# ververica/ForSt

Measured on AMD Instinct MI355X. Metric: device-resident GiB/s checksummed (CRC32C/XXH3), 4–64 KiB blocks, 1/2/4/8 GPU, higher is better.
Workload: dtype u8; 1 GPU; C2: 1 M x 4 KiB kCRC32c compute+verify; blocks_per_gpu=1048576, blocks_total=1048576, checksum=kCRC32c, step=trailer pass (write side) + verify pass (read side), parallelism=byte-balanced block shards of one batch x1, no data-path collective

## Files before the change

forst_amd/csrc/crc32c.hip:

```cpp
#include "crc32c_tables.h"
#include "crc_lds.h"
#include "device_common.h"
#include "engine.h"
#include "stream_common.h"

namespace forst {
namespace {

constexpr uint32_t kRB = FORST_CRC_ROUND_BYTES;
constexpr uint32_t kWaves = 16;
constexpr uint32_t kThreads = kWaves * 64;
constexpr uint32_t kRep = 32;
constexpr uint32_t kOffJump = 4 * 256 * kRep;
constexpr uint32_t kOffTree = kOffJump + 1024;
constexpr uint32_t kLdsDwords = kOffTree + FORST_CRC_TREE_LEVELS * 1024;
constexpr uint32_t kSmall = 32;

static_assert(kLdsDwords * 4 <= 160 * 1024, "CRC tables must fit in LDS");

__device__ __forceinline__ uint32_t lds_at(const uint32_t* __restrict__ L,
                                           uint32_t byte_addr) {
  return L[byte_addr >> 2];
}

__device__ __forceinline__ uint32_t crc_g(const uint32_t* __restrict__ L,
                                          uint32_t lb, uint32_t v) {
  const uint32_t a0 = ((v & 0xffu) << 7) + lb;
  const uint32_t a1 = (((v >> 8) & 0xffu) << 7) + lb;
  const uint32_t a2 = (((v >> 16) & 0xffu) << 7) + lb;
  const uint32_t a3 = ((v >> 24) << 7) + lb;
  return L[(a0 >> 2)] ^ L[(a1 >> 2) + 8192] ^ L[(a2 >> 2) + 16384] ^
         L[(a3 >> 2) + 24576];
}

__device__ __forceinline__ uint32_t crc_byte(const uint32_t* __restrict__ L,
                                             uint32_t lb, uint32_t s,
                                             uint32_t byte) {
  const uint32_t a = (((s ^ byte) & 0xffu) << 7) + lb;
  return L[(a >> 2) + 24576] ^ (s >> 8);
}

__device__ __forceinline__ uint32_t crc_shift(const uint32_t* __restrict__ L,
                                              uint32_t T, uint32_t v) {
  return L[T + (v & 0xffu)] ^ L[T + 256 + ((v >> 8) & 0xffu)] ^
         L[T + 512 + ((v >> 16) & 0xffu)] ^ L[T + 768 + (v >> 24)];
}

__device__ __forceinline__ void load_seg(uint32_t (&w)[16],
                                         const uint8_t* seg) {
#pragma unroll
  for (int k = 0; k < 4; ++k) {
    const u32x4a4 v = ld16_a4(seg + 16 * k);
    w[4 * k + 0] = v.x;
    w[4 * k + 1] = v.y;
    w[4 * k + 2] = v.z;
    w[4 * k + 3] = v.w;
  }
}

__device__ __forceinline__ void load_seg_checked(uint32_t (&w)[16],
                                                 const uint8_t* seg,
                                                 uint64_t lo) {
#pragma unroll
  for (int k = 0; k < 4; ++k) {
    const uint8_t* c = seg + 16 * k;
    const uint64_t ca = reinterpret_cast<uint64_t>(c);
    if (ca >= lo) {
      const u32x4a4 v = ld16_a4(c);
      w[4 * k + 0] = v.x;
      w[4 * k + 1] = v.y;
      w[4 * k + 2] = v.z;
      w[4 * k + 3] = v.w;
    } else {
#pragma unroll
      for (int d = 0; d < 4; ++d)
        w[4 * k + d] = (ca + 4 * d >= lo) ? ld4_a4(c + 4 * d) : 0u;
    }
  }
}

__device__ __forceinline__ uint32_t wave_crc32c(const uint32_t* __restrict__ L,
                                                uint32_t lane,
                                uint32_t lb, const uint8_t* p, uint64_t len,
                                uint32_t init, uint32_t nextra, uint32_t extra,
                                uint64_t lo) {
  uint32_t s;
  if (len < kSmall) {
    s = ~init;
    for (uint32_t i = 0; i < static_cast<uint32_t>(len); ++i)
      s = crc_byte(L, lb, s, ldu8(p + i));
  } else {
    const uint64_t A = reinterpret_cast<uint64_t>(p);
    const uint64_t E = A + len;
    const uint64_t Aal = A & ~3ull;
    const uint32_t m = static_cast<uint32_t>(A & 3);
    uint64_t Wend = E & ~3ull;
    const uint64_t D = Wend - Aal;
    uint32_t R = static_cast<uint32_t>((D + kRB - 1) / kRB);
    if (R > 1 && (D % kRB) == 4) {
      Wend -= 4;
      --R;
    }
    const uint64_t Wstart = Wend - static_cast<uint64_t>(R) * kRB;
    const uint32_t hA = static_cast<uint32_t>(Aal - Wstart);
    const uint32_t LA = hA >> 6;
    const uint32_t jA = (hA >> 2) & 15u;
    const uint8_t* seg = p - static_cast<int64_t>(A - Wstart) + lane * 64;

    uint32_t w[16];
    if (Wstart >= lo)
      load_seg(w, seg);
    else
      load_seg_checked(w, seg, lo);
    s = 0;
#pragma unroll
    for (int j = 0; j < 16; ++j) {
      if (static_cast<uint32_t>(j) == jA) {
        if (m == 0) {
          const uint32_t s0 = (lane == LA) ? ~init : s;
          s = crc_g(L, lb, s0 ^ w[j]);
        } else {
          const uint32_t sn = crc_g(L, lb, s ^ w[j]);
          uint32_t sb = ~init;
          uint32_t wb = w[j] >> (8 * m);
          for (uint32_t b = m; b < 4; ++b) {
            sb = crc_byte(L, lb, sb, wb & 0xffu);
            wb >>= 8;
          }
          s = (lane == LA) ? sb : sn;
        }
      } else {
        s = crc_g(L, lb, s ^ w[j]);
      }
    }
    s = (lane < LA) ? 0u : s;

    for (uint32_t r = 1; r < R; ++r) {
      seg += kRB;
      load_seg(w, seg);
      s = crc_shift(L, kOffJump, s);
#pragma unroll
      for (int j = 0; j < 16; ++j) s = crc_g(L, lb, s ^ w[j]);
    }

#pragma unroll
    for (int k = 0; k < FORST_CRC_TREE_LEVELS; ++k) {
      const uint32_t other = __shfl_xor(s, 1 << k);
      const bool right = (lane >> k) & 1;
      const uint32_t left_v = right ? other : s;
      const uint32_t right_v = right ? s : other;
      s = crc_shift(L, kOffTree + 1024u * k, left_v) ^ right_v;
    }

    const uint8_t* t = p + (Wend - A);
    const uint32_t nt = static_cast<uint32_t>(E - Wend);
    for (uint32_t i = 0; i < nt; ++i) s = crc_byte(L, lb, s, ldu8(t + i));
  }
  if (nextra) s = crc_byte(L, lb, s, extra);
  return ~s;
}

__device__ __forceinline__ void fill_tables(uint32_t* L) {
  const uint32_t tid = threadIdx.x;
  for (uint32_t i = tid; i < 4 * 256 * kRep; i += kThreads) L[i] = kCrcG[i >> 5];
  for (uint32_t i = tid; i < 1024; i += kThreads) L[kOffJump + i] = kCrcJump[i];
  for (uint32_t i = tid; i < FORST_CRC_TREE_LEVELS * 1024; i += kThreads)
    L[kOffTree + i] = kCrcTree[i];
  __syncthreads();
}

using namespace fcrc;
constexpr uint32_t kOffA2 = 65536;
constexpr uint32_t kOffB2 = kOffA2 + 15 * 4096;
constexpr uint32_t kSeg2 = FORST_CRC2_SEG_BYTES;

__device__ __forceinline__ uint32_t unstep_m(uint32_t v, uint32_t m) {
  if (m == 0) return v;
  const uint32_t* col = kCrcUnstep + 32 * (m - 1);
  uint32_t r = 0;
  for (uint32_t i = 0; i < 32; ++i) r ^= ((v >> i) & 1u) ? col[i] : 0u;
  return r;
}

template <int MODE>
__device__ __forceinline__ bool mem_last_byte(const BlockArgs& a) {
  return MODE == kModeVerify || ((MODE == kModeCompute || MODE == kModeTrailer) && !a.last_bytes);
}

__device__ __forceinline__ uint32_t small_crc2(const uint8_t* __restrict__ Lb, const Lanes& K,
                                               const uint8_t* p, uint32_t len, uint32_t init,
                                               uint32_t nextra, uint32_t extra) {
  uint32_t s = ~init;
  const uint32_t m = static_cast<uint32_t>(reinterpret_cast<uint64_t>(p) & 3);
  uint32_t nh = (4 - m) & 3;
  nh = nh < len ? nh : len;
  uint32_t y = 0;
  for (uint32_t i = 0; i < nh; ++i) y |= ldu8(p + i) << (8 * i);
  s = step_k(Lb, K, s, y, nh);
  uint32_t i = nh;
  for (; i + 4 <= len; i += 4) s = rep_map<false>(Lb, K, s ^ ld4v(p + i));
  y = 0;
  const uint32_t nt = len - i;
  for (uint32_t j = 0; j < nt; ++j) y |= ldu8(p + i + j) << (8 * j);
  s = step_k(Lb, K, s, y, nt);
  if (nextra) s = step_k(Lb, K, s, extra & 0xffu, 1);
  return ~s;
}

constexpr uint32_t kStageW = 6144;
constexpr uint32_t kRowRound = 1024;
constexpr uint32_t kRowChain = 512;
constexpr uint32_t kLds3Bytes = kOffB2 + 4096;
constexpr uint32_t kNoBlk = 0xffffffffu;

template <uint32_t NT>
__device__ __forceinline__ void fill_tables3(uint32_t* L) {
  const uint32_t tid = threadIdx.x;
  constexpr uint32_t kN1 = (16384 + NT - 1) / NT, kN2 = (15 * 1024 + NT - 1) / NT,
                     kN3 = (1024 + NT - 1) / NT;
  uint32_t v1[kN1], v2[kN2], v3[kN3];
#pragma unroll
  for (uint32_t k = 0; k < kN1; ++k) {
    const uint32_t i = tid + k * NT;
    const uint32_t e = (i >> 6) & 255, d = i & 63, t = (d >> 3) & 3;
    v1[k] = i < 16384 ? (d < 32 ? kCrcG[t * 256 + e] : kCrcJ3[t * 256 + e]) : 0u;
  }
#pragma unroll
  for (uint32_t k = 0; k < kN2; ++k) {
    const uint32_t i = tid + k * NT;
    v2[k] = i < 15 * 1024 ? kCrcA[i] : 0u;
  }
#pragma unroll
  for (uint32_t k = 0; k < kN3; ++k) {
    const uint32_t i = tid + k * NT;
    v3[k] = i < 1024 ? kCrcB[i] : 0u;
  }
#pragma unroll
  for (uint32_t k = 0; k < kN1; ++k)
    if (tid + k * NT < 16384) L[tid + k * NT] = v1[k];
#pragma unroll
  for (uint32_t k = 0; k < kN2; ++k)
    if (tid + k * NT < 15 * 1024) L[kOffA2 / 4 + tid + k * NT] = v2[k];
#pragma unroll
  for (uint32_t k = 0; k < kN3; ++k)
    if (tid + k * NT < 1024) L[kOffB2 / 4 + tid + k * NT] = v3[k];
  __syncthreads();
}

struct CRowPos {
  uint32_t rp_lo, rp_hi;
  uint32_t tp_lo, tp_hi;
  uint32_t rel;
  uint32_t rl;
  uint32_t pk;
  __device__ __forceinline__ int64_t rp() const {
    return static_cast<int64_t>((static_cast<uint64_t>(rp_hi) << 32) | rp_lo);
  }
  __device__ __forceinline__ uint64_t tp() const {
    return (static_cast<uint64_t>(tp_hi) << 32) | tp_lo;
  }
  __device__ __forceinline__ uint32_t cA() const { return pk & 1u; }
  __device__ __forceinline__ uint32_t tA() const { return (pk >> 1) & 15u; }
  __device__ __forceinline__ uint32_t jA() const { return (pk >> 5) & 7u; }
  __device__ __forceinline__ uint32_t q() const { return (pk >> 8) & 7u; }
  __device__ __forceinline__ uint32_t nt() const { return (pk >> 11) & 3u; }
  __device__ __forceinline__ uint32_t m() const { return (pk >> 13) & 3u; }
  __device__ __forceinline__ bool valid() const { return (pk >> 15) & 1u; }
  __device__ __forceinline__ bool slow() const { return (pk >> 16) & 1u; }
  __device__ __forceinline__ bool xtra() const { return (pk >> 17) & 1u; }
  __device__ __forceinline__ uint32_t d1() const { return (pk >> 16) & 12u; }
  __device__ __forceinline__ bool r0() const { return (pk >> 20) & 1u; }
  __device__ __forceinline__ uint32_t slow_size() const { return (pk >> 24) & 15u; }
  __device__ __forceinline__ bool wait() const { return (pk >> 21) & 1u; }
  template <int MODE>
  __device__ __forceinline__ uint64_t end(bool mlb) const {
    const uint64_t t0 = tp() + 4;
    const uint64_t we = (MODE == kModeVerify || nt() > 0) ? t0 : t0 + 4;
    return we + nt() - (mlb ? 1u : 0u);
  }
};

template <int MODE>
__device__ __forceinline__ void crow_derive(const BlockArgs& a, uint64_t off, uint32_t size,
                                            CRowPos& P) {
  const bool valid = P.rel != kNoBlk && desc_in_range<MODE>(a, Desc{off, size, 0, 0});
  const uint64_t E = off + size + (mem_last_byte<MODE>(a) ? 1u : 0u);
  const uint64_t ws = off & ~3ull;
  const uint64_t we = E & ~3ull;
  const uint64_t d4 = we - ws;
  const bool xtra = MODE != kModeRaw && (d4 & (kRowRound - 1)) == 4 && d4 > kRowRound;
  uint32_t R = static_cast<uint32_t>(xtra ? d4 / kRowRound : (d4 + kRowRound - 1) / kRowRound);
  int64_t w0 = static_cast<int64_t>(we) - (xtra ? 4 : 0) - static_cast<int64_t>(R) * kRowRound;
  const uint32_t hA = static_cast<uint32_t>(static_cast<int64_t>(ws) - w0);
  const uint32_t cA = hA >> 9, tA = (hA >> 5) & 15u, jA = (hA >> 2) & 7u;
  const int64_t seg_head = static_cast<int64_t>(ws) - 4 * static_cast<int64_t>(jA);
  const uint32_t q = seg_head < 0 ? static_cast<uint32_t>(-seg_head) >> 2 : 0u;
  const uint32_t nt = static_cast<uint32_t>(E - we);
  const uint32_t m = static_cast<uint32_t>(off & 3);
  const uint64_t t0 = (nt > 0 || MODE == kModeVerify) ? we : we - 4;
  const uint32_t d1 = MODE == kModeVerify ? (nt > 0 ? 8u : 4u) : (xtra && nt > 0 ? 0u : 4u);
  const bool slow = !valid || d4 < 4 || t0 < 4;
  const uint64_t tp = slow ? off : t0 - 4;
  if (slow) {
    R = 1;
    w0 = 0;
  }
  P.rl = R;
  P.rp_lo = static_cast<uint32_t>(w0);
  P.rp_hi = static_cast<uint32_t>(static_cast<uint64_t>(w0) >> 32);
  P.tp_lo = static_cast<uint32_t>(tp);
  P.tp_hi = static_cast<uint32_t>(tp >> 32);
  P.pk = (slow ? (valid ? (size & 15u) << 24 : 0u)
               : (cA | (tA << 1) | (jA << 5) | (q << 8) | (xtra ? 1u << 17 : 0u) |
                  ((d1 >> 2) << 18))) |
         (nt << 11) | (m << 13) | (valid ? 1u << 15 : 0u) | (slow ? 1u << 16 : 0u) | (1u << 20);
}

struct CRStep {
  uint32_t w[2][8];
  uint32_t t0, t1, t2, mod, extra;
};

template <int MODE>
__device__ __forceinline__ void crow_issue(const BlockArgs& a, uint32_t lane, const CRowPos& P,
                                           uint64_t kbeg, CRStep& d) {
  const uint32_t t = lane & 15;
  int64_t s0 = P.rp() + kSeg2 * t;
  int64_t s1 = s0 + kRowChain;
  if (__ballot(s0 < 0)) {
    s0 = s0 < 0 ? 0 : s0;
    s1 = s1 < 0 ? 0 : s1;
  }
#pragma unroll
  for (uint32_t c = 0; c < 2; ++c) {
    const uint8_t* sp = a.base + (c ? s1 : s0);
#pragma unroll
    for (int q = 0; q < 2; ++q) {
      const u32x4a4 v = ld16_a4(sp + 16 * q);
      d.w[c][4 * q + 0] = v.x;
      d.w[c][4 * q + 1] = v.y;
      d.w[c][4 * q + 2] = v.z;
      d.w[c][4 * q + 3] = v.w;
    }
  }
  const bool lastr = !P.slow() && P.rl <= 1;
  const uint8_t* pb = a.base + (lastr ? P.tp() : 0);
  d.t0 = ld4_a4(pb + 4);
  d.t1 = MODE == kModeRaw ? 0u : ld4_a4(pb + P.d1());
  d.t2 = MODE == kModeVerify ? ld4_a4(pb) : 0u;
  const uint64_t idx = kbeg + (P.rel == kNoBlk ? 0 : P.rel);
  if (MODE != kModeRaw)
    d.mod = a.modifiers ? a.modifiers[idx] : 0u;
  else
    d.mod = a.expect ? a.expect[idx] : 0u;
  if (MODE == kModeRaw)
    d.extra = a.init_crcs ? a.init_crcs[idx] : 0u;
  else if (MODE != kModeVerify)
    d.extra = a.last_bytes ? a.last_bytes[idx] : 0u;
  else
    d.extra = 0u;
}

constexpr uint32_t kRawSplit = 256;

__device__ __forceinline__ bool raw_long(uint64_t off, uint32_t size) {
  return size >= kRawSplit && (off >> 58) == 0;
}

template <int MODE, bool RAW_WG = false, bool FILT = false>
__device__ __forceinline__ void crc32c_rows_body(const BlockArgs& a) {
  static_assert(!FILT || (MODE == kModeRaw && !RAW_WG), "length split: raw global feed only");
  __shared__ uint32_t L[kLds3Bytes / 4];
  feed_init();
  fill_tables3<kThreads>(L);
  const uint8_t* Lb = reinterpret_cast<const uint8_t*>(L);
  const uint32_t lane = threadIdx.x & 63;
  const uint32_t wave = uniform(threadIdx.x >> 6);
  const uint32_t t = lane & 15;
  const Lanes K = lanes(lane);
  __shared__ uint32_t s0t[4];
  if (threadIdx.x < 4) s0t[threadIdx.x] = kCrcS0[threadIdx.x];
  __syncthreads();
  const uint64_t nw = static_cast<uint64_t>(gridDim.x) * kWaves;
  const uint64_t gw = static_cast<uint64_t>(blockIdx.x) * kWaves + wave;
  const bool has_extra = (MODE == kModeCompute || MODE == kModeTrailer) && a.last_bytes;

  BatchFeed feed;
  constexpr bool kWgFeed = MODE != kModeRaw || RAW_WG;
  constexpr uint32_t kChunk = 4;
  uint64_t cg = feed_first<kWgFeed, kChunk>(a, nw, gw, lane, feed);
  constexpr bool kStage = MODE != kModeRaw;
  __shared__ uint32_t st_out[kStage ? kStageW : 1];
  __shared__ uint8_t st_ok[kStage ? kStageW : 4];
  constexpr bool kRing = MODE == kModeRaw;
  constexpr uint32_t kRingN = 224;
  __shared__ uint32_t ring_i[kRing ? kWaves * kRingN : 1], ring_v[kRing ? kWaves * kRingN : 1];
  uint32_t* const ri = ring_i + (kRing ? wave * kRingN : 0);
  uint32_t* const rv = ring_v + (kRing ? wave * kRingN : 0);
  uint32_t rcount = 0;
  auto ring_flush = [&]() {
    wave_lds_sync();
    for (uint32_t j = lane; j < rcount; j += 64) a.out32[ri[j]] = rv[j];
    wave_lds_sync();
    rcount = 0;
  };
  if (!kStage && cg >= a.n) return;
  uint32_t clen = feed.len;
  uint64_t ng = 0;
  uint32_t nlen = 0;
  if constexpr (!FILT) {
    ng = feed_next<kWgFeed, kChunk>(a, nw, lane, feed);
    nlen = feed.len;
  }
  DescBatch cb, nb;
  uint64_t kbrel = 0;
  auto load_f = [&](uint64_t& g, uint32_t& len, DescBatch& d) {
    load_batch<MODE>(a, g, a.n, lane, d);
    if constexpr (FILT) {
      for (;;) {
        const bool keep =
            lane < len && raw_long((static_cast<uint64_t>(d.off_hi) << 32) | d.off_lo, d.size);
        const uint64_t km = __ballot(keep);
        if (km != 0 || len == 0) {
          batch_compact<false, false>(d, km, keep, lane);
          len = static_cast<uint32_t>(__popcll(km));
          break;
        }
        g = feed_next<kWgFeed, kChunk>(a, nw, lane, feed);
        len = feed.len;
        load_batch<MODE>(a, g, a.n, lane, d);
      }
    }
  };
  load_f(cg, clen, cb);
  if constexpr (FILT) {
    ng = feed_next<kWgFeed, kChunk>(a, nw, lane, feed);
    nlen = feed.len;
  }
  load_f(ng, nlen, nb);
  const uint64_t kbeg = 0;
  auto fetch = [&](uint64_t rel, CRowPos& P) {
    const BatchSlot q = batch_slot(rel, kbrel, cg, clen, ng, nlen, a.n);
    const uint32_t lo_c = __shfl(cb.off_lo, q.src), hi_c = __shfl(cb.off_hi, q.src);
    const uint32_t sz_c = __shfl(cb.size, q.src);
    const uint32_t lo_n = __shfl(nb.off_lo, q.src), hi_n = __shfl(nb.off_hi, q.src);
    const uint32_t sz_n = __shfl(nb.size, q.src);
    uint32_t hi = q.in_n ? hi_n : hi_c;
    uint64_t gi = q.gi;
    if constexpr (FILT) {
      gi = (q.in_n ? ng : cg) + (hi >> 26);
      hi &= 0x03ffffffu;
    }
    const uint64_t off = (static_cast<uint64_t>(hi) << 32) | (q.in_n ? lo_n : lo_c);
    const uint32_t size = q.in_n ? sz_n : sz_c;
    P.rel = q.valid ? static_cast<uint32_t>(gi) : kNoBlk;
    crow_derive<MODE>(a, off, size, P);
  };
  uint64_t next = 4;
  CRowPos C;
  fetch(lane >> 4, C);
  if constexpr (FILT) {
    const uint64_t avail = clen + nlen;
    if ((lane >> 4) >= avail && nlen != 0) C.pk |= 1u << 21;
    next = avail < 4 ? avail : 4;
  }
  auto advance = [&](const CRowPos& P, CRowPos& I) {
    const bool more = P.rel != kNoBlk && !P.slow() && P.rl > 1;
    const bool need = (P.rel != kNoBlk || (FILT && P.wait())) && !more;
    const uint64_t rows = __ballot(need && t == 0);
    I = P;
    if (more) {
      I.rl = P.rl - 1;
      I.pk = P.pk & ~(1u << 20);
      const int64_t rp = P.rp() + kRowRound;
      I.rp_lo = static_cast<uint32_t>(rp);
      I.rp_hi = static_cast<uint32_t>(static_cast<uint64_t>(rp) >> 32);
    }
    if (rows) {
      const uint32_t below = __builtin_amdgcn_mbcnt_hi(
          static_cast<uint32_t>(rows >> 32), __builtin_amdgcn_mbcnt_lo(static_cast<uint32_t>(rows), 0u));
      const uint32_t rank = below - (t != 0 && need ? 1u : 0u);
      CRowPos F;
      fetch(next + rank, F);
      uint64_t got = static_cast<uint64_t>(__popcll(rows));
      if constexpr (FILT) {
        const uint64_t avail = kbrel + clen + nlen - next;
        if (got > avail) got = avail;
        if (rank >= avail && nlen != 0) F.pk |= 1u << 21;
      }
      next += got;
      if (need) I = F;
      if (next >= kbrel + clen) {
        kbrel += clen;
        clen = nlen;
        cb = nb;
#ifndef FORST_HOST_EMULATION
        asm volatile("" : "+v"(cb.off_lo), "+v"(cb.off_hi), "+v"(cb.size));
#endif
        cg = ng;
        ng = feed_next<kWgFeed, kChunk>(a, nw, lane, feed);
        nlen = feed.len;
        load_f(ng, nlen, nb);
      }
    }
  };
  CRowPos I;
  advance(C, I);
  CRStep X, Y;
  crow_issue<MODE>(a, lane, C, kbeg, X);
  uint32_t s[2] = {0, 0};

  auto step = [&](CRStep& cu, CRStep& nx) -> bool {
    const bool live = __ballot(C.rel != kNoBlk || (FILT && C.wait())) != 0;
    if (MODE != kModeRaw && !live) return false;
    crow_issue<MODE>(a, lane, I, kbeg, nx);
    const bool fast = C.rel != kNoBlk && !C.slow();
    const bool r0 = C.r0();
    const bool head = __ballot(fast && r0);
    if (!head) {
#pragma unroll
      for (int c = 0; c < 2; ++c) {
        uint32_t lj[4], lg[4];
        look<true>(Lb, K, r0 ? 0u : s[c], lj);
        look<false>(Lb, K, cu.w[c][0], lg);
        uint32_t x = xor3(xor3(lj[0], lj[1], lj[2]), xor3(lj[3], lg[0], lg[1]),
                          xor3(lg[2], lg[3], cu.w[c][1]));
#pragma unroll
        for (int j = 2; j < 8; ++j) x = g_then(Lb, K, x, cu.w[c][j]);
        s[c] = g_then(Lb, K, x, 0u);
      }
    } else {
      const uint32_t cA = C.cA(), tA = C.tA(), jA = C.jA(), q = C.q(), m = C.m();
      const uint32_t bm = 0xffffffffu << (8 * m);
      const uint32_t S0 = MODE == kModeRaw && a.init_crcs ? unstep_m(~cu.extra, m) : s0t[m];
#pragma unroll
      for (uint32_t c = 0; c < 2; ++c) {
        const bool hl = fast && r0 && c == cA && t == tA;
        const bool pre = fast && r0 && (c < cA || (c == cA && t < tA));
        const uint32_t hj = hl ? jA : 8u;
        uint32_t wc[8];
#pragma unroll
        for (int j = 0; j < 8; ++j) wc[j] = cu.w[c][j];
        if (__ballot(hl && q != 0)) {
          uint32_t sh[8];
#pragma unroll
          for (int j = 0; j < 8; ++j) {
            uint32_t v = 0;
#pragma unroll
            for (int qq = 1; qq < 8; ++qq)
              if (qq <= j) v = (q == static_cast<uint32_t>(qq)) ? wc[j - qq] : v;
            sh[j] = v;
          }
#pragma unroll
          for (int j = 0; j < 8; ++j) wc[j] = (hl && q != 0) ? sh[j] : wc[j];
        }
        uint32_t lj[4], lg[4];
        look<true>(Lb, K, r0 ? 0u : s[c], lj);
        look<false>(Lb, K, hj == 0 ? ((wc[0] & bm) ^ S0) : wc[0], lg);
        uint32_t x = xor3(xor3(lj[0], lj[1], lj[2]), xor3(lj[3], lg[0], lg[1]),
                          xor3(lg[2], lg[3], wc[1]));
        x = hj == 1 ? ((wc[1] & bm) ^ S0) : x;
#pragma unroll
        for (uint32_t j = 2; j < 8; ++j) {
          x = g_then(Lb, K, x, wc[j]);
          x = hj == j ? ((wc[j] & bm) ^ S0) : x;
        }
        s[c] = pre ? 0u : g_then(Lb, K, x, 0u);
      }
    }
    const bool fin = C.rel != kNoBlk && (C.slow() || C.rl <= 1);
    if (__ballot(fin)) {
      const bool lo0 = t == 15;
      const uint32_t abase = kOffA2 + 4096 * (14 - t);
      uint32_t a0 = lo0 ? s[0] : shift_at(Lb, abase, s[0]);
      uint32_t a1 = lo0 ? s[1] : shift_at(Lb, abase, s[1]);
      a0 = row_ror_xor<1>(a0);
      a1 = row_ror_xor<1>(a1);
      a0 = row_ror_xor<2>(a0);
      a1 = row_ror_xor<2>(a1);
      a0 = row_ror_xor<4>(a0);
      a1 = row_ror_xor<4>(a1);
      a0 = row_ror_xor<8>(a0);
      a1 = row_ror_xor<8>(a1);
      uint32_t crc = 0, stored = 0;
      const uint32_t nt = C.nt();
      const bool calc = fin && (MODE == kModeTrailer ? t >= 11 : lo0);
      if (calc) {
        uint32_t st = shift_at(Lb, kOffB2, a0) ^ a1;
        if (MODE != kModeRaw && C.xtra()) st = step_k(Lb, K, st, MODE == kModeVerify ? cu.t2 : cu.t1, 4);
        uint32_t y = nt ? (cu.t0 & (0xffffffffu >> (32 - 8 * nt))) : 0u;
        uint32_t k = nt;
        if (has_extra) {
          y |= (cu.extra & 0xffu) << (8 * k);
          ++k;
        }
        crc = ~step_k(Lb, K, st, y, k);
        if (MODE == kModeVerify) stored = nt ? __builtin_amdgcn_alignbyte(cu.t1, cu.t0, nt) : cu.t0;
      }
      if (calc && C.slow() && C.valid()) {
        const uint8_t* pp = a.base + C.tp();
        const uint32_t init = MODE == kModeRaw ? cu.extra : 0u;
        crc = small_crc2(Lb, K, pp, C.slow_size() + (mem_last_byte<MODE>(a) ? 1u : 0u), init,
                         has_extra ? 1u : 0u, cu.extra);
        if (MODE == kModeVerify) stored = retire(ldu32(pp + C.slow_size() + 1));
        crc = retire(crc);
      }
      const bool valid = C.valid();
      const bool mine = fin && lo0;
      const uint64_t i = kbeg + (C.rel == kNoBlk ? 0 : C.rel);
      bool ok = valid;
      if (MODE == kModeRaw) {
        const uint32_t v = a.wal_hs ? crc_mask(crc) : crc;
        const bool differs = !a.expect || !valid || v != cu.mod;
        if constexpr (kRing) {
          const bool put = mine && differs && a.out32 != nullptr;
          const uint64_t pm = __ballot(put);
          if (pm) {
            const uint32_t at = rcount + __builtin_amdgcn_mbcnt_hi(
                static_cast<uint32_t>(pm >> 32), __builtin_amdgcn_mbcnt_lo(static_cast<uint32_t>(pm), 0u));
            if (put) {
              ri[at] = static_cast<uint32_t>(i);
              rv[at] = valid ? v : 0u;
            }
            rcount += static_cast<uint32_t>(__popcll(pm));
            if (rcount > kRingN - 64) ring_flush();
          }
        }
      } else if (MODE == kModeVerify) {
        const uint32_t computed = crc_mask(crc);
        const uint32_t st = stored - cu.mod;
        ok = valid && st == computed;
        const uint64_t sj = i - feed.wlo;
        const bool staged = kStage && sj < kStageW;
        if (mine && staged) {
          st_out[sj] = valid ? computed : 0u;
          st_ok[sj] = ok ? 1 : 0;
        }
        if (mine && !staged && a.out32) a.out32[i] = valid ? computed : 0u;
        if (mine && a.stored_out) a.stored_out[i] = valid ? st : 0u;
        if (mine && !staged && a.ok_out) a.ok_out[i] = ok ? 1 : 0;
        if (staged) ok = true;
      } else {
        const uint32_t out = crc_mask(crc) + cu.mod;
        const uint64_t sj = i - feed.wlo;
        const bool staged = kStage && sj < kStageW;
        if (mine && staged) {
          st_out[sj] = valid ? out : 0u;
          st_ok[sj] = valid ? 1 : 0;
        }
        if (mine && !staged && a.out32) a.out32[i] = valid ? out : 0u;
        if (MODE == kModeTrailer) {
          const uint32_t k = t - 11;
          if (!staged && calc && valid && (k != 0 || a.last_bytes)) {
            uint8_t* pw = a.base_w + (C.slow() ? C.tp() + C.slow_size()
                                               : C.template end<MODE>(mem_last_byte<MODE>(a)));
            pw[k] = static_cast<uint8_t>(k == 0 ? cu.extra : out >> (8 * (k - 1)));
          }
        }
      }
      if (MODE == kModeVerify) {
        const uint64_t badm = __ballot(mine && !ok);
        if (a.mismatches && badm && lane == 0)
          atomicAdd(a.mismatches, static_cast<unsigned long long>(__popcll(badm)));
      }
    }
#ifndef FORST_HOST_EMULATION
    asm volatile("" ::"v"(cu.t0), "v"(cu.t1), "v"(cu.t2), "v"(cu.mod), "v"(cu.extra));
#endif
    C = I;
    advance(C, I);
    return live;
  };
  if (MODE == kModeRaw) {
    for (bool more = true; more;) {
      step(X, Y);
      more = step(Y, X);
    }
  } else {
    while (step(X, Y) && step(Y, X)) {
    }
  }
  if constexpr (kRing) {
    if (rcount) ring_flush();
  }
  if constexpr (kStage) {
    __syncthreads();
    const uint64_t lo = feed.wlo, hi = feed.whi;
    const uint64_t m = hi > lo ? (hi - lo < kStageW ? hi - lo : kStageW) : 0;
    uint32_t bad = 0;
    for (uint32_t j = threadIdx.x; j < m; j += blockDim.x) {
      const uint64_t g = lo + j;
      if (a.out32) a.out32[g] = st_out[j];
      if (MODE == kModeVerify) {
        if (a.ok_out) a.ok_out[g] = st_ok[j];
        bad += st_ok[j] ? 0u : 1u;
      }
      if (MODE == kModeTrailer && st_ok[j]) {
        uint8_t* pw = a.base_w + a.offsets[g] + a.sizes[g];
        const uint32_t v = st_out[j];
        if (a.last_bytes) pw[0] = a.last_bytes[g];
        pw[1] = static_cast<uint8_t>(v);
        pw[2] = static_cast<uint8_t>(v >> 8);
        pw[3] = static_cast<uint8_t>(v >> 16);
        pw[4] = static_cast<uint8_t>(v >> 24);
      }
    }
    if (MODE == kModeVerify && a.mismatches) {
      uint32_t wb = bad;
#pragma unroll
      for (int o = 32; o > 0; o >>= 1) wb += __shfl_xor(wb, o);
      if (lane == 0 && wb) atomicAdd(a.mismatches, static_cast<unsigned long long>(wb));
    }
  }
}

template <int MODE>
__global__ void __launch_bounds__(kThreads) crc32c_rows_kernel(BlockArgs a) {
  crc32c_rows_body<MODE>(a);
}
__global__ void __launch_bounds__(kThreads) crc32c_rows_raw_small_kernel(BlockArgs a) {
  crc32c_rows_body<kModeRaw, true>(a);
}
__global__ void __launch_bounds__(kThreads) crc32c_rows_raw_filt_kernel(BlockArgs a) {
  crc32c_rows_body<kModeRaw, false, true>(a);
}

constexpr uint32_t kLaneThreads = 512;
constexpr uint32_t kLaneChunks = (kRawSplit + 2 + 4 + 15) / 16;
__device__ __forceinline__ uint32_t lane_raw_crc(const uint8_t* __restrict__ Lb, const Lanes& K,
                                                 const uint8_t* base, uint64_t base_len,
                                                 uint64_t off, uint32_t n, uint32_t init,
                                                 bool has_init) {
  const uint32_t m = static_cast<uint32_t>(off & 3);
  const uint32_t tot = n + m;
  const uint32_t nd = tot >> 2, nt = tot & 3;
  const uint32_t nc = (nd + (nt ? 1u : 0u) + 3) >> 2;
  if (nd == 0 || (off - m) + 16ull * nc > base_len)
    return small_crc2(Lb, K, base + off, n, init, 0, 0);
  const uint8_t* q = base + (off - m);
  const uint32_t S0 = has_init ? unstep_m(~init, m)
                               : m == 0 ? 0xffffffffu : m == 1 ? 0xa942e6bcu
                               : m == 2 ? 0x2804363bu : 0x96db52a8u;
  const uint32_t bm = 0xffffffffu << (8 * m);
  const uint32_t tm = (1u << (8 * nt)) - 1u;
  uint32_t s = 0;
  u32x4a4 v[kLaneChunks];
#pragma unroll
  for (uint32_t c = 0; c < kLaneChunks; ++c)
    v[c] = c < nc ? ld16_a4(q + 16 * c) : u32x4a4{0u, 0u, 0u, 0u};
#pragma unroll
  for (uint32_t c = 0; c < kLaneChunks; ++c) {
    if (c < nc) {
      const uint32_t w[4] = {v[c].x, v[c].y, v[c].z, v[c].w};
#pragma unroll
      for (uint32_t j = 0; j < 4; ++j) {
        const uint32_t i = 4 * c + j;
        if (i < nd)
          s = rep_map<false>(Lb, K, i == 0 ? ((w[j] & bm) ^ S0) : (s ^ w[j]));
        else if (i == nd && nt)
          s = step_k(Lb, K, s, w[j] & tm, nt);
      }
    }
  }
  return ~s;
}

constexpr uint32_t kRawLaneR = 4;
constexpr uint32_t kRawLaneWaves = kLaneThreads / 64;
__global__ void __launch_bounds__(kLaneThreads) crc32c_raw_lane_kernel(BlockArgs a) {
  __shared__ uint32_t L[16384];
  __shared__ uint16_t slot[kRawLaneWaves][kRawLaneR * 64];
  for (uint32_t i = threadIdx.x; i < 16384; i += kLaneThreads) {
    const uint32_t e = i >> 6, d = i & 63;
    if (d < 32) L[i] = kCrcG[((d >> 3) & 3) * 256 + e];
  }
  __syncthreads();
  const uint8_t* Lb = reinterpret_cast<const uint8_t*>(L);
  const uint32_t lane = threadIdx.x & 63;
  const uint32_t wave = uniform(threadIdx.x >> 6);
  const Lanes K = lanes(lane);
  const uint64_t below = (1ull << lane) - 1;
  const uint64_t nw = static_cast<uint64_t>(gridDim.x) * kRawLaneWaves;
  constexpr uint64_t W = uint64_t(kRawLaneR) * 64;
  uint16_t* sl = slot[wave];
  for (uint64_t w0 = (static_cast<uint64_t>(blockIdx.x) * kRawLaneWaves + wave) * W; w0 < a.n;
       w0 += nw * W) {
    uint32_t olo[kRawLaneR], ohi[kRawLaneR], sz[kRawLaneR];
#pragma unroll
    for (uint32_t r = 0; r < kRawLaneR; ++r) {
      uint64_t i = w0 + 64 * r + lane;
      i = i < a.n ? i : a.n - 1;
      const uint64_t off = a.offsets[i];
      olo[r] = static_cast<uint32_t>(off);
      ohi[r] = static_cast<uint32_t>(off >> 32);
      sz[r] = a.sizes[i];
    }
    uint32_t cnt = 0;
#pragma unroll
    for (uint32_t r = 0; r < kRawLaneR; ++r) {
      uint64_t off = (static_cast<uint64_t>(ohi[r]) << 32) | olo[r];
      uint32_t size = sz[r];
      if (a.wal_hs) {
        const bool ok = off <= a.base_len && a.base_len - off >= uint64_t(a.wal_hs) + size;
        off = ok ? off + 6 : ~0ull;
        size = ok ? a.wal_hs + size - 6 : 0u;
        olo[r] = static_cast<uint32_t>(off);
        ohi[r] = static_cast<uint32_t>(off >> 32);
        sz[r] = size;
      }
      const bool sh = w0 + 64 * r + lane < a.n && !raw_long(off, size);
      const uint64_t m = __ballot(sh);
      if (sh) sl[cnt + static_cast<uint32_t>(__popcll(m & below))] = static_cast<uint16_t>(64 * r + lane);
      cnt += static_cast<uint32_t>(__popcll(m));
    }
    wave_lds_sync();
    for (uint32_t j0 = 0; j0 < cnt; j0 += 64) {
      const uint32_t j = j0 + lane;
      const uint32_t q = j < cnt ? sl[j] : 0u;
      const int src = static_cast<int>(4 * (q & 63));
      uint32_t lo = 0, hi = 0, size = 0;
#pragma unroll
      for (uint32_t r = 0; r < kRawLaneR; ++r) {
        const uint32_t vlo = static_cast<uint32_t>(__builtin_amdgcn_ds_bpermute(src, static_cast<int>(olo[r])));
        const uint32_t vhi = static_cast<uint32_t>(__builtin_amdgcn_ds_bpermute(src, static_cast<int>(ohi[r])));
        const uint32_t vsz = static_cast<uint32_t>(__builtin_amdgcn_ds_bpermute(src, static_cast<int>(sz[r])));
        if ((q >> 6) == r) {
          lo = vlo;
          hi = vhi;
          size = vsz;
        }
      }
      if (j < cnt) {
        const uint64_t i = w0 + q;
        const uint64_t off = (static_cast<uint64_t>(hi) << 32) | lo;
        const bool valid = desc_in_range<kModeRaw>(a, Desc{off, size, 0, 0});
        const uint32_t init = a.init_crcs ? a.init_crcs[i] : 0u;
        uint32_t v = 0;
        if (valid) {
          const uint32_t crc = lane_raw_crc(Lb, K, a.base, a.base_len, off, size, init,
                                            a.init_crcs != nullptr);
          v = a.wal_hs ? crc_mask(crc) : crc;
        }
        const bool differs = !a.expect || !valid || v != a.expect[i];
        if (differs && a.out32) a.out32[i] = v;
      }
    }
    wave_lds_sync();
  }
}

template <int MODE>
__global__ void __launch_bounds__(kThreads)
    crc32c_block_kernel_simple(BlockArgs a) {
  __shared__ uint32_t L[kLdsDwords];
  fill_tables(L);
  const uint32_t lane = threadIdx.x & 63;
  const uint32_t wave = uniform(threadIdx.x >> 6);
  const uint32_t lb = (lane & 31) << 2;
  const uint64_t lo = reinterpret_cast<uint64_t>(a.base);
  const uint64_t nw = static_cast<uint64_t>(gridDim.x) * kWaves;
  for (uint64_t i = static_cast<uint64_t>(blockIdx.x) * kWaves + wave; i < a.n;
       i += nw) {
    const uint64_t off = a.offsets[i];
    const uint32_t size = a.sizes[i];
    const uint8_t* p = a.base + off;
    uint64_t need = size;
    if (MODE == kModeVerify || MODE == kModeTrailer) need += 5;
    if (MODE == kModeCompute && a.last_bytes == nullptr) need += 1;
    const bool inb = off <= a.base_len && need <= a.base_len - off;
    if (!inb) {
      if (lane == 0) {
        if (a.out32) a.out32[i] = 0;
        if (MODE == kModeVerify) {
          if (a.ok_out) a.ok_out[i] = 0;
          if (a.stored_out) a.stored_out[i] = 0;
          if (a.mismatches) atomicAdd(a.mismatches, 1ull);
        }
      }
      continue;
    }
    if (MODE == kModeRaw) {
      const uint32_t init = a.init_crcs ? a.init_crcs[i] : 0u;
      const uint32_t c = wave_crc32c(L, lane, lb, p, size, init, 0, 0, lo);
      if (lane == 0) a.out32[i] = c;
    } else if (MODE == kModeVerify) {
      const uint32_t computed =
          crc_mask(wave_crc32c(L, lane, lb, p, uint64_t(size) + 1, 0, 0, 0, lo));
      const uint32_t mod = a.modifiers ? a.modifiers[i] : 0u;
      const uint32_t stored = ldu32(p + size + 1) - mod;
      const bool ok = stored == computed;
      if (lane == 0) {
        if (a.out32) a.out32[i] = computed;
        if (a.stored_out) a.stored_out[i] = stored;
        if (a.ok_out) a.ok_out[i] = ok ? 1 : 0;
        if (!ok && a.mismatches) atomicAdd(a.mismatches, 1ull);
      }
    } else {
      const uint32_t last = a.last_bytes ? a.last_bytes[i] : ldu8(p + size);
      const uint32_t mod = a.modifiers ? a.modifiers[i] : 0u;
      const uint32_t c =
          crc_mask(wave_crc32c(L, lane, lb, p, size, 0, 1, last, lo)) + mod;
      if (lane == 0) {
        if (a.out32) a.out32[i] = c;
        if (MODE == kModeTrailer) {
          uint8_t* q = a.base_w + off + size;
          q[0] = static_cast<uint8_t>(last);
          stu32_bytes(q + 1, c);
        }
      }
    }
  }
}

}

namespace {

enum class CrcKernel {
  kSimple,
  kRows,
};

hipError_t launch_kernel(void (*k)(BlockArgs), uint32_t grid, uint32_t threads, BlockArgs a,
                         hipStream_t s) {
  hipLaunchKernelGGL(k, dim3(grid), dim3(threads), 0, s, a);
  return hipGetLastError();
}

const char* crc_kernel_name(CrcKernel k, int mode) {
  static const char* const kNames[][4] = {
      {"crc32c_block_kernel_simple<compute>", "crc32c_block_kernel_simple<trailer>",
       "crc32c_block_kernel_simple<verify>", "crc32c_block_kernel_simple<raw>"},
      {"crc32c_rows_kernel<compute>", "crc32c_rows_kernel<trailer>", "crc32c_rows_kernel<verify>",
       "crc32c_rows_kernel<raw>"},
  };
  return kNames[static_cast<int>(k)][mode & 3];
}

#ifndef FORST_CRC_BLOCK_COST
#define FORST_CRC_BLOCK_COST 0
#endif
template <int M>
hipError_t launch_crc_mode(CrcKernel k, const BlockArgs& a, uint32_t grid, hipStream_t s) {
  switch (k) {
    case CrcKernel::kSimple:
      return launch_kernel(crc32c_block_kernel_simple<M>, grid, kThreads, a, s);
    case CrcKernel::kRows:
      if constexpr (M != kModeRaw) {
        BlockArgs b = a;
        b.wg_cost = FORST_CRC_BLOCK_COST;
        return launch_kernel(crc32c_rows_kernel<M>, grid, 64 * kWaves, b, s);
      } else {
        if (a.n < uint64_t(64) * grid * kWaves)
          return launch_kernel(crc32c_rows_raw_small_kernel, grid, 64 * kWaves, a, s);
        const hipError_t e = launch_kernel(crc32c_raw_lane_kernel, 2 * device_info().num_cus,
                                           kLaneThreads, a, s);
        if (e != hipSuccess) return e;
        return launch_fed(crc32c_rows_raw_filt_kernel, grid, kWaves, a, s);
      }
  }
  return hipErrorInvalidValue;
}

hipError_t launch_crc32c_slice(int mode, const BlockArgs& a, hipStream_t stream,
                               const char** name) {
  const DeviceInfo& di = device_info();
  uint32_t grid = static_cast<uint32_t>(std::min<uint64_t>((a.n + kWaves - 1) / kWaves, di.num_cus));
  if (grid == 0) grid = 1;
#ifdef FORST_DEBUG_BOUNDS
  {
    DbgState st{};
    st.lo = reinterpret_cast<uint64_t>(a.base);
    st.hi = st.lo + a.base_len;
    hipError_t e = hipMemcpyToSymbolAsync(HIP_SYMBOL(g_forst_dbg), &st, sizeof(st), 0,
                                          hipMemcpyHostToDevice, stream);
    if (e != hipSuccess) return e;
  }
#endif
  const CrcKernel k = a.base_len < kRB ? CrcKernel::kSimple : CrcKernel::kRows;
  if (a.wal_hs && (mode != kModeRaw || k != CrcKernel::kRows)) return hipErrorInvalidValue;
  *name = crc_kernel_name(k, mode);
  if (k == CrcKernel::kRows && mode == kModeRaw)
    *name = a.n < uint64_t(64) * grid * kWaves ? "crc32c_rows_raw_small_kernel"
                                               : "crc32c_rows_raw_filt_kernel";
  switch (mode) {
    case kModeCompute:
      return launch_crc_mode<kModeCompute>(k, a, grid, stream);
    case kModeTrailer:
      return launch_crc_mode<kModeTrailer>(k, a, grid, stream);
    case kModeVerify:
      return launch_crc_mode<kModeVerify>(k, a, grid, stream);
    default:
      return launch_crc_mode<kModeRaw>(k, a, grid, stream);
  }
}

}

hipError_t launch_crc32c_raw_lanes(const BlockArgs& a, hipStream_t stream) {
  if (a.n == 0) return hipSuccess;
  return launch_kernel(crc32c_raw_lane_kernel, 2 * device_info().num_cus, kLaneThreads, a, stream);
}

hipError_t launch_crc32c_blocks(int mode, const BlockArgs& a, hipStream_t stream,
                                const char** name) {
  for (uint64_t first = 0; first < a.n; first += FORST_ROWS_MAX_DESCS) {
    const BlockArgs b = slice_descs(a, first, std::min<uint64_t>(a.n - first, FORST_ROWS_MAX_DESCS));
    const hipError_t e = launch_crc32c_slice(mode, b, stream, name);
    if (e != hipSuccess) return e;
  }
  return hipSuccess;
}

}

#ifdef FORST_DEBUG_BOUNDS
extern "C" __attribute__((visibility("default"))) int forst_debug_fetch(unsigned long long* out) {
  forst::DbgState st{};
  if (hipMemcpyFromSymbol(&st, HIP_SYMBOL(forst::g_forst_dbg), sizeof(st)) != hipSuccess)
    return -3;
  for (int k = 0; k < 4; ++k) out[k] = st.rec[k];
  return 0;
}
#endif
```

forst_amd/csrc/stream_common.h:

```cpp
#pragma once
#include "device_common.h"
#include "engine.h"

namespace forst {

constexpr uint32_t kBatch = 64;

__device__ __forceinline__ uint32_t readlane32(uint32_t v, uint32_t l) {
  return static_cast<uint32_t>(__builtin_amdgcn_readlane(static_cast<int>(v), static_cast<int>(l)));
}
__device__ __forceinline__ uint64_t readlane64(uint32_t lo, uint32_t hi, uint32_t l) {
  return (static_cast<uint64_t>(readlane32(hi, l)) << 32) | readlane32(lo, l);
}


__device__ __forceinline__ void wave_share(uint64_t n, uint64_t nw, uint64_t gw, uint64_t& kbeg,
                                           uint64_t& kend) {
  const uint64_t q = n / nw, rem = n % nw;
  kbeg = gw * q + (gw < rem ? gw : rem);
  kend = kbeg + q + (gw < rem ? 1 : 0);
}

struct BatchFeed {
  uint64_t g;
  uint64_t lim;
  uint64_t rr;
  uint64_t wlo, whi;
  uint32_t len;
};

__device__ __forceinline__ void feed_set_len(const BlockArgs& a, BatchFeed& f) {
  const uint64_t e = f.lim < a.n ? f.lim : a.n;
  const uint64_t l = f.g < e ? e - f.g : 0;
  f.len = static_cast<uint32_t>(l < kBatch ? l : kBatch);
}

__device__ __forceinline__ uint64_t feed_claim_global(const BlockArgs& a, uint64_t nw,
                                                      uint32_t lane, BatchFeed& f) {
  uint64_t t;
  if (a.ticket) {
    const uint32_t l = lane + vzero();
    const unsigned long long v = atomicAdd(a.ticket + l, l == 0 ? 1ull : 0ull);
    t = uniform64(v);
  } else {
    t = f.rr;
    f.rr += nw;
  }
  f.g = nw * a.share1 + static_cast<uint64_t>(kBatch) * t;
  f.lim = f.g + kBatch;
  feed_set_len(a, f);
  return f.g;
}

constexpr uint32_t kWgChunk = 16;
__device__ __forceinline__ uint32_t* feed_lds_ctr() {
  __shared__ uint32_t ctr;
  return &ctr;
}
__device__ __forceinline__ void feed_init() {
  if (threadIdx.x == 0) *feed_lds_ctr() = 0;
}

__device__ __forceinline__ uint64_t frac_point(uint64_t off0, uint64_t span, uint64_t b,
                                               uint64_t G) {
  return off0 + (span / G) * b + ((span % G) * b) / G;
}

__device__ __forceinline__ void wg_range(const BlockArgs& a, uint32_t lane, uint64_t* lo_out,
                                         uint64_t* hi_out) {
  const uint64_t n = a.n, G = gridDim.x, b = blockIdx.x;
  const uint64_t c = a.wg_cost;
  const uint64_t off0 = a.offsets[0];
  const uint64_t last = a.offsets[n - 1] + a.sizes[n - 1] + c * (n - 1);
  if (last <= off0 || G == 1) {
    const uint64_t W = (n + G - 1) / G;
    *lo_out = b * W < n ? b * W : n;
    *hi_out = (b + 1) * W < n ? (b + 1) * W : n;
    return;
  }
  const uint64_t span = last - off0;
  const uint64_t t0 = frac_point(off0, span, b, G), t1 = frac_point(off0, span, b + 1, G);
  uint64_t lo0 = 0, len0 = n, lo1 = 0, len1 = n;
  while (len0 > 64 || len1 > 64) {
    const uint64_t st0 = (len0 + 63) / 64, st1 = (len1 + 63) / 64;
    const uint64_t q0 = lo0 + lane * st0, q1 = lo1 + lane * st1;
    const bool v0 = len0 > 64 && lane > 0 && q0 < lo0 + len0;
    const bool v1 = len1 > 64 && lane > 0 && q1 < lo1 + len1;
    const uint64_t k0 = a.offsets[v0 ? q0 : 0] + c * q0, k1 = a.offsets[v1 ? q1 : 0] + c * q1;
    const uint64_t c0 = static_cast<uint64_t>(__popcll(__ballot(v0 && k0 < t0)));
    const uint64_t c1 = static_cast<uint64_t>(__popcll(__ballot(v1 && k1 < t1)));
    if (len0 > 64) {
      const uint64_t e = lo0 + len0;
      lo0 += c0 * st0;
      len0 = e - lo0 < st0 ? e - lo0 : st0;
    }
    if (len1 > 64) {
      const uint64_t e = lo1 + len1;
      lo1 += c1 * st1;
      len1 = e - lo1 < st1 ? e - lo1 : st1;
    }
  }
  const bool f0 = lane < len0, f1 = lane < len1;
  const uint64_t k0 = a.offsets[f0 ? lo0 + lane : 0] + c * (lo0 + lane),
                 k1 = a.offsets[f1 ? lo1 + lane : 0] + c * (lo1 + lane);
  const uint64_t L0 = lo0 + static_cast<uint64_t>(__popcll(__ballot(f0 && k0 < t0)));
  const uint64_t L1 = lo1 + static_cast<uint64_t>(__popcll(__ballot(f1 && k1 < t1)));
  *lo_out = b == 0 ? 0 : uniform64(L0);
  *hi_out = b + 1 == G ? n : uniform64(L1);
}

template <uint32_t CHUNK>
__device__ __forceinline__ uint64_t feed_claim_wg(const BlockArgs& a, uint32_t lane,
                                                  BatchFeed& f) {
  uint32_t p = 0;
  if (lane == 0) p = atomicAdd(feed_lds_ctr(), CHUNK);
  p = readlane32(p, 0);
  f.g = f.wlo + p;
  if (f.g >= f.whi) {
    f.g = a.n;
    f.len = 0;
  } else {
    f.len = static_cast<uint32_t>(f.whi - f.g < CHUNK ? f.whi - f.g : CHUNK);
  }
  f.lim = f.g + f.len;
  return f.g;
}

template <bool WG, uint32_t CHUNK = kWgChunk>
__device__ __forceinline__ uint64_t feed_first(const BlockArgs& a, uint64_t nw, uint64_t gw,
                                               uint32_t lane, BatchFeed& f) {
  f.rr = gw;
  if (WG) {
    wg_range(a, lane, &f.wlo, &f.whi);
    return feed_claim_wg<CHUNK>(a, lane, f);
  }
  if (a.share1 == 0) return feed_claim_global(a, nw, lane, f);
  f.g = gw * a.share1;
  f.lim = f.g + a.share1;
  feed_set_len(a, f);
  return f.g;
}

template <bool WG, uint32_t CHUNK = kWgChunk>
__device__ __forceinline__ uint64_t feed_next(const BlockArgs& a, uint64_t nw, uint32_t lane,
                                              BatchFeed& f) {
  if (f.g >= a.n) {
    f.len = 0;
    return f.g;
  }
  if (WG) return feed_claim_wg<CHUNK>(a, lane, f);
  f.g += kBatch;
  if (f.g < f.lim) {
    feed_set_len(a, f);
    return f.g;
  }
  return feed_claim_global(a, nw, lane, f);
}

struct BatchSlot {
  int src;
  bool in_n, valid;
  uint64_t gi;
};
__device__ __forceinline__ BatchSlot batch_slot(uint64_t rel, uint64_t kbrel, uint64_t cg,
                                                uint32_t clen, uint64_t ng, uint32_t nlen,
                                                uint64_t n) {
  const uint32_t j = static_cast<uint32_t>(rel - kbrel);
  BatchSlot b;
  b.in_n = j >= clen;
  const uint32_t k = b.in_n ? j - clen : j;
  b.src = static_cast<int>(k & 63u);
  b.gi = (b.in_n ? ng : cg) + k;
  b.valid = k < (b.in_n ? nlen : clen) && b.gi < n;
  return b;
}

struct DescBatch {
  uint32_t off_lo, off_hi, size, mod, extra;
};

template <int MODE>
__device__ __forceinline__ void load_batch(const BlockArgs& a, uint64_t kb, uint64_t kend,
                                           uint32_t lane, DescBatch& d) {
  uint64_t i = kb + lane;
  i = i < kend ? i : kend - 1;
  uint64_t off = a.offsets[i];
  uint32_t size = a.sizes[i];
  if (MODE == kModeRaw && a.wal_hs) {
    const bool ok = off <= a.base_len && a.base_len - off >= uint64_t(a.wal_hs) + size;
    off = ok ? off + 6 : ~0ull;
    size = ok ? a.wal_hs + size - 6 : 0u;
  }
  d.off_lo = static_cast<uint32_t>(off);
  d.off_hi = static_cast<uint32_t>(off >> 32);
  d.size = size;
  const uint32_t* mp = a.modifiers ? a.modifiers : a.sizes;
  const uint32_t mv = mp[i];
  d.mod = a.modifiers ? mv : 0u;
  if (MODE == kModeRaw) {
    const uint32_t* ip = a.init_crcs ? a.init_crcs : a.sizes;
    const uint32_t iv = ip[i];
    d.extra = a.init_crcs ? iv : 0u;
  } else {
    const uint8_t* lp = a.last_bytes ? a.last_bytes : reinterpret_cast<const uint8_t*>(a.sizes);
    d.extra = lp[i];
  }
}

__device__ __forceinline__ bool below_2p58(const DescBatch& d) { return (d.off_hi >> 26) == 0; }
template <bool EXTRA, bool MOD>
__device__ __forceinline__ void batch_compact(DescBatch& d, uint64_t km, bool keep,
                                              uint32_t lane) {
  const uint64_t below = (1ull << lane) - 1;
  const uint32_t nk = static_cast<uint32_t>(__popcll(km));
  const uint32_t dst = keep ? static_cast<uint32_t>(__popcll(km & below))
                            : nk + static_cast<uint32_t>(__popcll(~km & below));
  const int ad = static_cast<int>(4 * dst);
  auto perm = [&](uint32_t v) {
    return static_cast<uint32_t>(__builtin_amdgcn_ds_permute(ad, static_cast<int>(v)));
  };
  d.off_lo = perm(d.off_lo);
  d.off_hi = perm((d.off_hi & 0x03ffffffu) | (lane << 26));
  d.size = perm(d.size);
  if (EXTRA) d.extra = perm(d.extra);
  if (MOD) d.mod = perm(d.mod);
}

struct Desc {
  uint64_t off;
  uint32_t size, mod, extra;
};
__device__ __forceinline__ Desc batch_desc(uint64_t k, uint64_t kb, const DescBatch& cb,
                                           const DescBatch& nb) {
  const uint32_t kk = static_cast<uint32_t>(k - kb);
  const uint32_t sl = kk & 63u;
  const bool in_n = kk >= 64;
  Desc d;
  const uint64_t off_c = readlane64(cb.off_lo, cb.off_hi, sl);
  const uint64_t off_n = readlane64(nb.off_lo, nb.off_hi, sl);
  d.off = in_n ? off_n : off_c;
  const uint32_t size_c = readlane32(cb.size, sl), size_n = readlane32(nb.size, sl);
  d.size = in_n ? size_n : size_c;
  const uint32_t mod_c = readlane32(cb.mod, sl), mod_n = readlane32(nb.mod, sl);
  d.mod = in_n ? mod_n : mod_c;
  const uint32_t ex_c = readlane32(cb.extra, sl), ex_n = readlane32(nb.extra, sl);
  d.extra = in_n ? ex_n : ex_c;
  return d;
}

template <int MODE>
__device__ __forceinline__ bool desc_in_range(const BlockArgs& a, const Desc& d) {
  uint64_t need = d.size;
  if (MODE == kModeVerify || MODE == kModeTrailer) need += 5;
  if (MODE == kModeCompute && !a.last_bytes) need += 1;
  return d.off <= a.base_len && need <= a.base_len - d.off;
}

inline hipError_t launch_fed(void (*k)(BlockArgs), uint32_t grid, uint32_t waves, BlockArgs b,
                             hipStream_t s) {
  hipError_t e = feed_setup(b, uint64_t(grid) * waves, s);
  if (e != hipSuccess) return e;
  hipLaunchKernelGGL(k, dim3(grid), dim3(64 * waves), 0, s, b);
  e = hipGetLastError();
  const hipError_t f = scratch_free(b.ticket, s);
  return e != hipSuccess ? e : f;
}

}
```

Before: 5412 GiB/s.

## Overlap CRC table fill with first row issue in staged modes

For non-raw modes (compute/trailer/verify), the kernel now holds the LDS table values in registers and issues the first row's global loads before storing the tables to LDS and synchronizing. Each wave claims its first chunk statically (wave*kChunk), with the LDS counter pre-seeded, so no atomic is needed before the barrier. The second batch load and advance are deferred until after the sync. The aim is to hide kernel prologue latency (global table reads, barrier, descriptor fetch) behind the first data loads. In exchange, register pressure rises because the table values are held across the issue, and lanes beyond the chunk length are clamped to redundant descriptor loads.

```diff
diff --git a/forst_amd/csrc/crc32c.hip b/forst_amd/csrc/crc32c.hip
--- a/forst_amd/csrc/crc32c.hip
+++ b/forst_amd/csrc/crc32c.hip
@@ -214,11 +214,18 @@
 constexpr uint32_t kNoBlk = 0xffffffffu;
 
 template <uint32_t NT>
-__device__ __forceinline__ void fill_tables3(uint32_t* L) {
+struct TabRegs {
+  static constexpr uint32_t kN1 = (16384 + NT - 1) / NT, kN2 = (15 * 1024 + NT - 1) / NT,
+                            kN3 = (1024 + NT - 1) / NT;
+  uint32_t v1[kN1], v2[kN2], v3[kN3];
+};
+template <uint32_t NT>
+__device__ __forceinline__ void tab_load(TabRegs<NT>& r) {
   const uint32_t tid = threadIdx.x;
-  constexpr uint32_t kN1 = (16384 + NT - 1) / NT, kN2 = (15 * 1024 + NT - 1) / NT,
-                     kN3 = (1024 + NT - 1) / NT;
-  uint32_t v1[kN1], v2[kN2], v3[kN3];
+  constexpr uint32_t kN1 = TabRegs<NT>::kN1, kN2 = TabRegs<NT>::kN2, kN3 = TabRegs<NT>::kN3;
+  uint32_t(&v1)[kN1] = r.v1;
+  uint32_t(&v2)[kN2] = r.v2;
+  uint32_t(&v3)[kN3] = r.v3;
 #pragma unroll
   for (uint32_t k = 0; k < kN1; ++k) {
     const uint32_t i = tid + k * NT;
@@ -235,6 +242,14 @@
     const uint32_t i = tid + k * NT;
     v3[k] = i < 1024 ? kCrcB[i] : 0u;
   }
+}
+template <uint32_t NT>
+__device__ __forceinline__ void tab_store(uint32_t* L, const TabRegs<NT>& r) {
+  const uint32_t tid = threadIdx.x;
+  constexpr uint32_t kN1 = TabRegs<NT>::kN1, kN2 = TabRegs<NT>::kN2, kN3 = TabRegs<NT>::kN3;
+  const uint32_t(&v1)[kN1] = r.v1;
+  const uint32_t(&v2)[kN2] = r.v2;
+  const uint32_t(&v3)[kN3] = r.v3;
 #pragma unroll
   for (uint32_t k = 0; k < kN1; ++k)
     if (tid + k * NT < 16384) L[tid + k * NT] = v1[k];
@@ -244,6 +259,12 @@
 #pragma unroll
   for (uint32_t k = 0; k < kN3; ++k)
     if (tid + k * NT < 1024) L[kOffB2 / 4 + tid + k * NT] = v3[k];
+}
+template <uint32_t NT>
+__device__ __forceinline__ void fill_tables3(uint32_t* L) {
+  TabRegs<NT> r;
+  tab_load(r);
+  tab_store(L, r);
   __syncthreads();
 }
 
@@ -371,24 +392,41 @@
 __device__ __forceinline__ void crc32c_rows_body(const BlockArgs& a) {
   static_assert(!FILT || (MODE == kModeRaw && !RAW_WG), "length split: raw global feed only");
   __shared__ uint32_t L[kLds3Bytes / 4];
-  feed_init();
-  fill_tables3<kThreads>(L);
+  constexpr bool kEarly = MODE != kModeRaw;
+  constexpr bool kWgFeed = MODE != kModeRaw || RAW_WG;
+  constexpr uint32_t kChunk = 4;
+  feed_init(kEarly ? kWaves * kChunk : 0);
+  TabRegs<kThreads> tabs;
+  uint32_t s0v = 0;
+  if constexpr (kEarly) {
+    tab_load(tabs);
+    s0v = kCrcS0[threadIdx.x & 3];
+  } else {
+    fill_tables3<kThreads>(L);
+  }
   const uint8_t* Lb = reinterpret_cast<const uint8_t*>(L);
   const uint32_t lane = threadIdx.x & 63;
   const uint32_t wave = uniform(threadIdx.x >> 6);
   const uint32_t t = lane & 15;
   const Lanes K = lanes(lane);
   __shared__ uint32_t s0t[4];
-  if (threadIdx.x < 4) s0t[threadIdx.x] = kCrcS0[threadIdx.x];
-  __syncthreads();
+  if constexpr (!kEarly) {
+    if (threadIdx.x < 4) s0t[threadIdx.x] = kCrcS0[threadIdx.x];
+    __syncthreads();
+  }
   const uint64_t nw = static_cast<uint64_t>(gridDim.x) * kWaves;
   const uint64_t gw = static_cast<uint64_t>(blockIdx.x) * kWaves + wave;
   const bool has_extra = (MODE == kModeCompute || MODE == kModeTrailer) && a.last_bytes;
 
   BatchFeed feed;
-  constexpr bool kWgFeed = MODE != kModeRaw || RAW_WG;
-  constexpr uint32_t kChunk = 4;
-  uint64_t cg = feed_first<kWgFeed, kChunk>(a, nw, gw, lane, feed);
+  uint64_t cg;
+  if constexpr (kEarly) {
+    feed.rr = gw;
+    wg_range(a, lane, &feed.wlo, &feed.whi);
+    cg = feed_take_wg<kChunk>(a, wave * kChunk, feed);
+  } else {
+    cg = feed_first<kWgFeed, kChunk>(a, nw, gw, lane, feed);
+  }
   constexpr bool kStage = MODE != kModeRaw;
   __shared__ uint32_t st_out[kStage ? kStageW : 1];
   __shared__ uint8_t st_ok[kStage ? kStageW : 4];
@@ -408,14 +446,14 @@
   uint32_t clen = feed.len;
   uint64_t ng = 0;
   uint32_t nlen = 0;
-  if constexpr (!FILT) {
+  if constexpr (!FILT && !kEarly) {
     ng = feed_next<kWgFeed, kChunk>(a, nw, lane, feed);
     nlen = feed.len;
   }
   DescBatch cb, nb;
   uint64_t kbrel = 0;
   auto load_f = [&](uint64_t& g, uint32_t& len, DescBatch& d) {
-    load_batch<MODE>(a, g, a.n, lane, d);
+    load_batch<MODE, kEarly ? kChunk : kBatch>(a, g, a.n, lane, d);
     if constexpr (FILT) {
       for (;;) {
         const bool keep =
@@ -437,7 +475,10 @@
     ng = feed_next<kWgFeed, kChunk>(a, nw, lane, feed);
     nlen = feed.len;
   }
-  load_f(ng, nlen, nb);
+  if constexpr (kEarly)
+    nb = cb;
+  else
+    load_f(ng, nlen, nb);
   const uint64_t kbeg = 0;
   auto fetch = [&](uint64_t rel, CRowPos& P) {
     const BatchSlot q = batch_slot(rel, kbrel, cg, clen, ng, nlen, a.n);
@@ -505,9 +546,20 @@
     }
   };
   CRowPos I;
-  advance(C, I);
   CRStep X, Y;
-  crow_issue<MODE>(a, lane, C, kbeg, X);
+  if constexpr (kEarly) {
+    crow_issue<MODE>(a, lane, C, kbeg, X);
+    tab_store(L, tabs);
+    if (threadIdx.x < 4) s0t[threadIdx.x] = s0v;
+    __syncthreads();
+    ng = feed_next<kWgFeed, kChunk>(a, nw, lane, feed);
+    nlen = feed.len;
+    load_f(ng, nlen, nb);
+    advance(C, I);
+  } else {
+    advance(C, I);
+    crow_issue<MODE>(a, lane, C, kbeg, X);
+  }
   uint32_t s[2] = {0, 0};
 
   auto step = [&](CRStep& cu, CRStep& nx) -> bool {
diff --git a/forst_amd/csrc/stream_common.h b/forst_amd/csrc/stream_common.h
--- a/forst_amd/csrc/stream_common.h
+++ b/forst_amd/csrc/stream_common.h
@@ -57,8 +57,8 @@
   __shared__ uint32_t ctr;
   return &ctr;
 }
-__device__ __forceinline__ void feed_init() {
-  if (threadIdx.x == 0) *feed_lds_ctr() = 0;
+__device__ __forceinline__ void feed_init(uint32_t first = 0) {
+  if (threadIdx.x == 0) *feed_lds_ctr() = first;
 }
 
 __device__ __forceinline__ uint64_t frac_point(uint64_t off0, uint64_t span, uint64_t b,
@@ -110,11 +110,7 @@
 }
 
 template <uint32_t CHUNK>
-__device__ __forceinline__ uint64_t feed_claim_wg(const BlockArgs& a, uint32_t lane,
-                                                  BatchFeed& f) {
-  uint32_t p = 0;
-  if (lane == 0) p = atomicAdd(feed_lds_ctr(), CHUNK);
-  p = readlane32(p, 0);
+__device__ __forceinline__ uint64_t feed_take_wg(const BlockArgs& a, uint32_t p, BatchFeed& f) {
   f.g = f.wlo + p;
   if (f.g >= f.whi) {
     f.g = a.n;
@@ -124,6 +120,13 @@
   }
   f.lim = f.g + f.len;
   return f.g;
+}
+template <uint32_t CHUNK>
+__device__ __forceinline__ uint64_t feed_claim_wg(const BlockArgs& a, uint32_t lane,
+                                                  BatchFeed& f) {
+  uint32_t p = 0;
+  if (lane == 0) p = atomicAdd(feed_lds_ctr(), CHUNK);
+  return feed_take_wg<CHUNK>(a, readlane32(p, 0), f);
 }
 
 template <bool WG, uint32_t CHUNK = kWgChunk>
@@ -179,10 +182,10 @@
   uint32_t off_lo, off_hi, size, mod, extra;
 };
 
-template <int MODE>
+template <int MODE, uint32_t LEN = kBatch>
 __device__ __forceinline__ void load_batch(const BlockArgs& a, uint64_t kb, uint64_t kend,
                                            uint32_t lane, DescBatch& d) {
-  uint64_t i = kb + lane;
+  uint64_t i = kb + (LEN < kBatch && lane >= LEN ? LEN - 1 : lane);
   i = i < kend ? i : kend - 1;
   uint64_t off = a.offsets[i];
   uint32_t size = a.sizes[i];
```

Result: no change. 5422 GiB/s (median of 6 runs) (+0.2%).
